# PrivEimantas/myFYP

Measured on AMD Instinct MI355X. Metric: rounds/sec + wall-clock-to-target-acc, MNIST MLP FedAvg 8 peers at 1/2/4/8 MI355X, higher is better.
Workload: dtype fp32

## Files before the change

csrc/kernels/mlp_persistent.h:

```cpp
#pragma once
#include "mlp_fused.h"

struct MLPPersistBufs {
  bf16* h1x;
  bf16* w2x;
  bf16* dh2x;
  unsigned* flags;
  size_t flag_bytes;
  int* err;
  int plain_ok;
  int plain;
};

bool mlp_persistent_supported(const MLPArgs& a);
size_t mlp_persistent_bytes(int P, int Bpad);
size_t mlp_persistent_flag_bytes(int P);
int mlp_persistent_blocks(int P);
hipError_t mlp_persistent_prepare(const MLPArgs& a);
hipError_t mlp_launch_persistent_epoch(const MLPArgs& a, const MLPPersistBufs& pb, hipStream_t s, bool zero_flags = true);

struct MLPPersistF32Bufs {
  float* h1x;
  float* plx;
  float* dh2x;
  unsigned* gen;
  unsigned* flags;
  size_t flag_bytes;
  int* err;
  unsigned fbase;
  float* w2chk;
  int plain_ok;
  int plain;
  int plain_x;
  int c2_straight;
  int k24;
};

int mlp_plain_pub_mode();
bool mlp_persistent_f32_supported(const MLPArgs& a);
size_t mlp_persistent_f32_h1x_floats(int P, int Bpad);
size_t mlp_persistent_f32_bytes(int P, int Bpad);
size_t mlp_persistent_f32_flag_bytes(int P);
int mlp_persistent_f32_gang();
int mlp_persistent_f32_resident_capacity(const MLPArgs& a, int num_cus);
int mlp_persistent_f32_launch_wgs(const MLPArgs& a);
int mlp_persistent_f32_ks(const MLPArgs& a);
int mlp_persistent_f32_variant(const MLPArgs& a);
int mlp_persistent_f32_flags_per_peer();
void mlp_persistent_f32_flag_layout(int* line, int* lines_per_peer, int* full_lines);
hipError_t mlp_persistent_f32_prepare(const MLPArgs& a);
hipError_t mlp_launch_persistent_f32_epoch(const MLPArgs& a, const MLPPersistF32Bufs& pb, hipStream_t s, bool zero_flags = true,
                                           const int* active = nullptr);
void mlp_launch_eval_f32(const MLPArgs& a, int max_rows, hipStream_t s);
```

csrc/kernels/mlp_persistent_f32.hip:

```cpp
#include <atomic>

#include "mlp_persistent.h"
#include "persist_common.h"
#include "mlp_f32_common.h"

bool mlp_f32v2_supported(const MLPArgs& a);
size_t mlp_f32v2_lds(const MLPArgs& a);
size_t mlp_f32v2_bytes(int P, int Bpad);
int mlp_f32v2_launch_wgs();
int mlp_f32v2_resident_capacity(const MLPArgs& a, int num_cus);
hipError_t mlp_f32v2_prepare(const MLPArgs& a);
void mlp_f32v2_launch(const MLPArgs& a, const MLPPersistF32Bufs& pb, hipStream_t s);

#ifdef MLP_STAMPS
__device__ unsigned long long g_p32_stamps[2][128][18];
__device__ unsigned long long g_p32_epoch[4];
#define P32_STAMP(role, t, i)                                                                    \
  do {                                                                                           \
    if (p == 0 && threadIdx.x == 0 && (t) < 128) g_p32_stamps[role][t][i] = wall_clock64(); \
  } while (0)
#define P32_ESTAMP(i)                                        \
  do {                                                       \
    if (p == 0 && threadIdx.x == 0) g_p32_epoch[i] = wall_clock64(); \
  } while (0)
// ... 183 lines not shown
    if (q == RQ && (KS != 1 || s >= KS1)) break;
#pragma unroll
    for (int half = 0; half < 2; ++half) {
      const int k = C0 + 32 * s + 16 * half + 4 * h;
      float4 wv = {0.f, 0.f, 0.f, 0.f}, mv = wv, vv = wv, ev = wv;
      if (s < KS1 && k < D0) {
        const int64_t idx = pS + a.off_w1 + (int64_t)orow * D0 + k;
        wv = *reinterpret_cast<const float4*>(a.params + idx);
        if (!fresh) {
          mv = *reinterpret_cast<const float4*>(a.m + idx);
          if (ADAM) vv = *reinterpret_cast<const float4*>(a.v + idx);
        }
        if (EXTRA) ev = float4{extra_at(a, idx), extra_at(a, idx + 1), extra_at(a, idx + 2), extra_at(a, idx + 3)};
      } else if (s < KS1 && k == D0) {
        const int64_t idx = pS + a.off_b1 + orow;
        wv.x = a.params[idx];
        if (!fresh) {
          mv.x = a.m[idx];
          if (ADAM) vv.x = a.v[idx];
        }
        if (EXTRA) ev.x = extra_at(a, idx);
      }
      if (q < RQ) {
        const float wa[4] = {wv.x, wv.y, wv.z, wv.w}, ma[4] = {mv.x, mv.y, mv.z, mv.w}, va[4] = {vv.x, vv.y, vv.z, vv.w},
                    ea[4] = {ev.x, ev.y, ev.z, ev.w};
#pragma unroll
        for (int i = 0; i < 4; ++i) {
          w1[q][4 * half + i] = wa[i];
          m1[q][4 * half + i] = ma[i];
          v1[q][4 * half + i] = va[i];
          e1[q][4 * half + i] = ea[i];
        }
      } else {
        const int off = c * 32 + 16 * half + 4 * h;
        *reinterpret_cast<float4*>(sW1x + off) = wv;
        *reinterpret_cast<float4*>(sW1x + 512 + off) = mv;
        *reinterpret_cast<float4*>(sW1x + 1024 + off) = vv;
        *reinterpret_cast<float4*>(sW1x + 1536 + off) = ev;
      }
    }
  }
  float w2c[4], m2c[4], v2c[4], e2c[4];
#pragma unroll
  for (int i = 0; i < 4; ++i) {
    const int64_t idx = pS + a.off_w2 + (int64_t)(16 * wave + 4 * h + i) * PD1 + NCG * cg + c;
    w2c[i] = a.params[idx];
    m2c[i] = fresh ? 0.f : a.m[idx];
    v2c[i] = (ADAM && !fresh) ? a.v[idx] : 0.f;
    e2c[i] = EXTRA ? extra_at(a, idx) : 0.f;
  }

  auto bias_chunk = [](bool valid) { return uint4{valid ? 0x3F80u : 0u, 0u, 0u, 0u}; };
  auto xw_stage = [&](int t, int lv) {
    const int rows = rows_at(a, n, t);
#pragma unroll
    for (int k = 0; k < XPT; ++k) {
      const int q = k / (BP / 16), kk = k % (BP / 16);
      if (q > RQ || (q == RQ && KS != 1)) break;
      const int s = wave + 8 * q;
      const int idx = kk * 64 + lv;
      const int r = idx >> 2, col = 32 * s + 8 * (idx & 3), gcol = C0 + col;
      if (s < KS1 && gcol < D0) {
        const bf16* src = a.Xb16 + ((int64_t)p * a.xb_rows + (int64_t)t * a.B + r) * D0 + gcol;
        *reinterpret_cast<uint4*>(sX + r * LDX + col) = r < rows ? *reinterpret_cast<const uint4*>(src) : uint4{0u, 0u, 0u, 0u};
      } else if (s < KS1 && gcol == D0) {
        *reinterpret_cast<uint4*>(sX + r * LDX + col) = bias_chunk(r < rows);
      }
    }
  };
  {
    const int z0 = D0 - C0 + 8, z1 = KS1 * 32;
    if (z0 < z1)
      for (int e = tid; e < BP * (z1 - z0); e += NT) {
        const int r = e / (z1 - z0), q = e % (z1 - z0);
        sX[r * LDX + (z0 + q)] = (bf16)0.f;
      }
  }
  if (nsteps > 0) xw_stage(0, lane);

  auto w2_replica_update = [&](int tp, float lr_p, float inv_p) {
    const __amdgpu_buffer_rsrc_t rd = rsrc_of(pb.dh2x + ((int64_t)p * 2 + (tp & 1)) * BP * PD2 * 2, BP * PD2 * 8);
    int lr = lane;
    asm volatile("" : "+v"(lr));
    const int ro = 4 * ((lr >> 4) * PD2 + 16 * wave + (lr & 15));
    const float* h1p = sH1 + (tp & 1) * BP * 16;
    float av[BP / 4];
#pragma unroll
    for (int kb = 0; kb < BP / 4; ++kb) av[kb] = __builtin_bit_cast(float, __builtin_amdgcn_raw_buffer_load_b32(rd, ro + 4 * 4 * kb * PD2, 0, 16));
    f32x4 acc = zero4();
#pragma unroll
    for (int kb = 0; kb < BP / 4; ++kb) acc = mfma_f32(av[kb], h1p[(4 * kb + h) * 16 + c], acc);
#pragma unroll
    for (int i = 0; i < 4; ++i) upd32<ADAM, EXTRA>(o, acc[i], w2c[i], m2c[i], v2c[i], e2c[i], lr_p, inv_p, wdmu);
  };
  auto fwd_kstep = [&](int q, f32x4(&acc)[MT], bool chk = true, bool rx = false) __attribute__((always_inline)) {
    const int s = wave + 8 * q;
    if (chk && s >= KS1) return;
    int lq = lane;
    asm volatile("" : "+v"(lq));
    const int hq = lq >> 4, cq = lq & 15;
    float wq[8];
#pragma unroll
    for (int j = 0; j < 8; ++j) wq[j] = q < RQ ? w1[q < RQ ? q : 0][j] : rx ? w1x[j] : sW1x[cq * 32 + kappa(hq, j)];
    bf16x8 bh, bm, bl;
    split3(wq, bh, bm, bl);
    if constexpr (FUSE) {
      bf16x8 af[MT];
#pragma unroll
      for (int mt = 0; mt < MT; ++mt) {
        const bf16* xp = sX + (16 * mt + cq) * LDX + 32 * s + 4 * (hq & 1);
        af[mt] = cat8(*reinterpret_cast<const bf16x4*>(xp + ((hq >> 1) << 3)), *reinterpret_cast<const bf16x4*>(xp + ((2 + (hq >> 1)) << 3)));
      }
#pragma unroll
      for (int mt = 0; mt < MT; ++mt) acc[mt] = mfma_bf16(af[mt], bl, acc[mt]);
#pragma unroll
      for (int mt = 0; mt < MT; ++mt) acc[mt] = mfma_bf16(af[mt], bm, acc[mt]);
#pragma unroll
      for (int mt = 0; mt < MT; ++mt) acc[mt] = mfma_bf16(af[mt], bh, acc[mt]);
      return;
    }
#pragma unroll
    for (int mt = 0; mt < MT; ++mt) {
      const bf16* xp = sX + (16 * mt + cq) * LDX + 32 * s + 4 * (hq & 1);
      const bf16x8 af = cat8(*reinterpret_cast<const bf16x4*>(xp + ((hq >> 1) << 3)), *reinterpret_cast<const bf16x4*>(xp + ((2 + (hq >> 1)) << 3)));
      acc[mt] = mfma3(af, bh, bm, bl, acc[mt]);
    }
  };
  auto fwd_all = [&](f32x4(&acc)[MT]) {
#pragma unroll
    for (int mt = 0; mt < MT; ++mt) acc[mt] = zero4();
#pragma unroll
    for (int q = 0; q < (KS == 1 ? RQ + 1 : RQ); ++q) {
      fwd_kstep(q, acc);
      __builtin_amdgcn_sched_barrier(0);
    }
  };
  auto h1_publish = [&](int t, const f32x4(&acc)[MT]) -> bool {
    const int rows = rows_at(a, n, t);
    float* sH1c = sH1 + (t & 1) * BP * 16;
    int tq = tid;
    asm volatile("" : "+v"(tq));
#pragma unroll
    for (int mt = 0; mt < MT; ++mt) sRed[(wave * MT + mt) * 64 + (tq & 63)] = acc[mt];
    lds_barrier();
    if (tq < MT * 64) {
      const int mt = tq >> 6, hh = (tq & 63) >> 4, cc = tq & 15;
      f32x4 s = sRed[mt * 64 + (tq & 63)];
#pragma unroll
      for (int w = 1; w < 8; ++w) s += sRed[(w * MT + mt) * 64 + (tq & 63)];
#pragma unroll
      for (int i = 0; i < 4; ++i) {
        const int b = 16 * mt + 4 * hh + i;
        const float v = b < rows ? (KS == 1 ? fmaxf(s[i], 0.f) : s[i]) : 0.f;
        sH1c[b * 16 + cc] = v;
        persist::pub32(pb.plain, h1x_part(pb, p, kh, t, BP) + (unsigned)(b * PD1 + NCG * cg + cc), v);
      }
    }
    if (g == 0) P32_STAMP(0, t, 1);
    persist::publish_p(pb.flags, FPP, p, XR ? F_H1P + cg * KS + kh : F_H1 + g, pb.fbase + (unsigned)(t + 1), pb.plain);
    if (XR) {
      if (!persist::wg_wait(pb.flags, FPP, p, F_H1P + cg * KS, KS, pb.fbase + (unsigned)(t + 1), pb.err, sOk)) return false;
      if (tid < BP * 4) {
        const int b = tid >> 2, c4 = 4 * (tid & 3);
        float4 u[KS];
#pragma unroll
        for (int k2 = 0; k2 < KS; ++k2)
          u[k2] = k2 == kh ? *reinterpret_cast<const float4*>(sH1c + b * 16 + c4)
                           : ld_sc1_16(rsrc_of(h1x_part(pb, p, k2, t, BP), BP * PD1 * 4), (b * PD1 + NCG * cg + c4) * 4);
        float4 sum = u[0];
#pragma unroll
        for (int k2 = 1; k2 < KS; ++k2) {
// ... 62 lines not shown
    const unsigned t1 = (unsigned)(t + 1);
    bc.next(o, lr_t, inv_bc2);
    float* sH1c = sH1 + (t & 1) * BP * 16;
    if (g == 0) P32_STAMP(0, t, 0);

    if constexpr (!FUSE) {
      f32x4 acc[MT];
      fwd_all(acc);
      if (g == 0) P32_STAMP(0, t, 7);
      if (!h1_publish(t, acc)) return;
    }

    if (!RH && t > 0) w2_replica_update(t - 1, lr_prev, inv_prev);
    if (g == 0) P32_STAMP(0, t, 3);

    const bool more = t + 1 < nsteps;
    if (more) {
      const int rows_n = rows_at(a, n, t + 1);
      unsigned sink = 0;
      int xi = lane;
      if (FUSE) asm volatile("" : "+v"(xi));
      const bf16* xbase = a.Xb16 + ((int64_t)p * a.xb_rows + (int64_t)(t + 1) * a.B) * D0;
      const bf16* xrow = xbase + (unsigned)(xi * D0);
#pragma unroll
      for (int q = 0; q < (KS == 1 ? RQ + 1 : RQ); ++q) {
        const int s = wave + 8 * q;
        const int r = lane;
        if (s < KS1 && C0 + 32 * s < D0 && r < rows_n && r < BP)
          sink ^= *reinterpret_cast<const unsigned*>(xrow + C0 + 32 * s);
      }
      asm volatile("" ::"v"(sink));
    }

    constexpr int XQF = FUSE ? BP / 16 : 1;
    uint4 xqf[XQF];
    const __amdgpu_buffer_rsrc_t r_xn =
        rsrc_of(a.Xb16 + ((int64_t)p * a.xb_rows + (int64_t)(t + 1) * a.B) * D0, more ? rows_at(a, n, t + 1) * D0 * 2 : 0);
    auto xq_load = [&](int q, bool chk = true) __attribute__((always_inline)) {
      const int s = wave + 8 * q;
      if (chk && s >= KS1) return;
      int lx = lane;
      if (chk)
        asm volatile("" : "+v"(lx));
      else
        lx = tv & 63;
#pragma unroll
      for (int kk = 0; kk < XQF; ++kk) {
        const int idx = kk * 64 + lx;
        const int r = idx >> 2, gcol = C0 + 32 * s + 8 * (idx & 3);
        unsigned off = (unsigned)(r * D0 + gcol) * 2u;
        asm("" : "+v"(off));
        off = gcol < D0 ? off : 0x7FFFFFF0u;
        asm("" : "+v"(off));
        xqf[kk] = __builtin_bit_cast(uint4, __builtin_amdgcn_raw_buffer_load_b128(r_xn, off, 0, 0));
      }
    };
    if constexpr (FUSE) xq_load(0);

    const float* dh2_t = pb.dh2x + ((int64_t)p * 2 + (t & 1)) * BP * PD2 * 2;
    const __amdgpu_buffer_rsrc_t r_dh2 = rsrc_of(dh2_t, BP * PD2 * 8);
    if (!persist::wg_wait(pb.flags, FPP, p, RH ? F3_DH2 : F_DH2, RH ? nhr_of(BP) : NH, pb.fbase + t1, pb.err, sOk)) return;
    if (g == 0) P32_STAMP(0, t, 4);
    if (KS > 1 && !XR) {
      if (tid < BP * 4) {
        const int b = tid >> 2, c4 = 4 * (tid & 3);
        float4 sum = {0.f, 0.f, 0.f, 0.f};
#pragma unroll
        for (int k2 = 0; k2 < KS; ++k2) {
          float4 v;
          if (k2 == kh) {
            v = *reinterpret_cast<const float4*>(sH1c + b * 16 + c4);
          } else {
            const __amdgpu_buffer_rsrc_t r = rsrc_of(h1x_part(pb, p, k2, t, BP), BP * PD1 * 4);
            v = ld_sc1_16(r, (b * PD1 + NCG * cg + c4) * 4);
          }
          sum.x += v.x;
          sum.y += v.y;
          sum.z += v.z;
          sum.w += v.w;
        }
        *reinterpret_cast<float4*>(sH1c + b * 16 + c4) = float4{fmaxf(sum.x, 0.f), fmaxf(sum.y, 0.f), fmaxf(sum.z, 0.f), fmaxf(sum.w, 0.f)};
      }
    }
    {
      float4 v[BP / 16];
#pragma unroll
      for (int k = 0; k < BP / 16; ++k) v[k] = ld_sc1_16(r_dh2, (tv + NT * k) * 16);
#pragma unroll
      for (int k = 0; k < BP / 16; ++k) {
        const int e = tv + NT * k;
        *reinterpret_cast<float4*>(sDH2 + (e >> 5) * LDD + 4 * (e & 31)) = v[k];
      }
    }
    lds_barrier();
    if (sOk[1] == 0) return;
    {
      f32x4 acc1[MT];
#pragma unroll
      for (int mt = 0; mt < MT; ++mt) {
        const float4 av = *reinterpret_cast<const float4*>(sDH2 + (16 * mt + c) * LDD + 16 * wave + 4 * h);
        f32x4 acc = mfma_f32(av.x, w2c[0], zero4());
        acc = mfma_f32(av.y, w2c[1], acc);
        acc = mfma_f32(av.z, w2c[2], acc);
        acc1[mt] = mfma_f32(av.w, w2c[3], acc);
      }
      f32x4 dw2 = zero4();
      if (RH) {
        const float* h1p = sH1c;
#pragma unroll
        for (int kb = 0; kb < BP / 4; ++kb) dw2 = mfma_f32(sDH2[(4 * kb + h) * LDD + 16 * wave + c], h1p[(4 * kb + h) * 16 + c], dw2);
      }
      lds_barrier();
#pragma unroll
      for (int mt = 0; mt < MT; ++mt) sRed[(wave * MT + mt) * 64 + lane] = acc1[mt];
      if (RH) {
#pragma unroll
        for (int i = 0; i < 4; ++i) upd32<ADAM, EXTRA>(o, dw2[i], w2c[i], m2c[i], v2c[i], e2c[i], lr_t, inv_bc2, wdmu);
        if (kh == 0) {
          float* w2x = pb.dh2x + (int64_t)a.P * 2 * BP * PD2 * 2 + (int64_t)p * PD2 * PD1;
#pragma unroll
          for (int i = 0; i < 4; ++i) persist::pub32(pb.plain, w2x + (16 * wave + 4 * h + i) * PD1 + NCG * cg + c, w2c[i]);
        }
      }
    }
    if (RH && kh == 0) {
      persist::publish_p(pb.flags, FPP, p, F3_W2 + cg, pb.fbase + (unsigned)(t + 2), pb.plain);
    } else {
      lds_barrier();
    }
    if (tv < MT * 64) {
      const int mt = tv >> 6, hh = (tv & 63) >> 4, cc = tv & 15;
      f32x4 s = sRed[mt * 64 + (tv & 63)];
#pragma unroll
      for (int w = 1; w < 8; ++w) s += sRed[(w * MT + mt) * 64 + (tv & 63)];
      bf16x4 dh, dm, dl;
#pragma unroll
      for (int i = 0; i < 4; ++i) {
        const float d = sH1c[(16 * mt + 4 * hh + i) * 16 + cc] > 0.f ? s[i] : 0.f;
        const bf16 x0 = (bf16)d;
        const float r = d - (float)x0;
        const bf16 x1 = (bf16)r;
        dh[i] = x0;
        dm[i] = x1;
        dl[i] = (bf16)(r - (float)x1);
      }
      const int off = cc * LDT + 16 * mt + 4 * hh;
      *reinterpret_cast<bf16x4*>(sD3 + off) = dh;
      *reinterpret_cast<bf16x4*>(sD3 + 16 * LDT + off) = dm;
      *reinterpret_cast<bf16x4*>(sD3 + 32 * LDT + off) = dl;
    }
    lds_barrier();
    if (g == 0) P32_STAMP(0, t, 5);
    {
      int lv = lane;
      asm volatile("" : "+v"(lv));
      f32x4 accF[FUSE ? MT : 1];
#pragma unroll
      for (int mt = 0; mt < (FUSE ? MT : 1); ++mt) accF[mt] = zero4();
      const int rows_next = more ? rows_at(a, n, t + 1) : 0;
      const bf16* xnext = a.Xb16 + ((int64_t)p * a.xb_rows + (int64_t)(t + 1) * a.B) * D0;
      constexpr int DFR = FUSE ? BP / 32 : 1;
      bf16x8 dfr[3][DFR];
      if (FUSE && ST) {
        int lq = lane;
        asm volatile("" : "+v"(lq));
        const bf16* dfrag = sD3 + (lq & 15) * LDT + 8 * (lq >> 4);
#pragma unroll
        for (int kb = 0; kb < DFR; ++kb) {
          dfr[0][kb] = ld8(dfrag + 32 * kb);
          dfr[1][kb] = ld8(dfrag + 16 * LDT + 32 * kb);
          dfr[2][kb] = ld8(dfrag + 32 * LDT + 32 * kb);
        }
      }
#pragma unroll
      for (int q = 0; q < QN; ++q) {
        if (q >= qn) continue;
        const bool STq = ST && (q < RQ || KR);
        const int s = wave + 8 * q;
        if (STq || s < KS1) {
          int lq = lane;
          asm volatile("" : "+v"(lq));
          const bf16* dfrag = sD3 + (lq & 15) * LDT + 8 * (lq >> 4);
          constexpr int XQ = BP / 16;
          uint4 xq[XQ];
#pragma unroll
          for (int kk = 0; kk < XQ; ++kk) {
            if constexpr (FUSE) {
              xq[kk] = xqf[FUSE ? kk : 0];
              continue;
            }
            const int idx = kk * 64 + lv;
            const int r = idx >> 2, col = 32 * s + 8 * (idx & 3), gcol = C0 + col;
            if (STq) {
              unsigned off = (unsigned)(r * D0 + gcol) * 2u;
              asm("" : "+v"(off));
// ... 301 lines not shown
          acc[mt] = mfma_f32(av.x, w2[gg][0], acc[mt]);
          acc[mt] = mfma_f32(av.y, w2[gg][1], acc[mt]);
          acc[mt] = mfma_f32(av.z, w2[gg][2], acc[mt]);
          acc[mt] = mfma_f32(av.w, w2[gg][3], acc[mt]);
        }
      }
#pragma unroll
      for (int mt = 0; mt < MT; ++mt) sRed[(wave * MT + mt) * 64 + lane] = acc[mt];
    }
    lds_barrier();
    if (tid < MT * 64) {
      const int mt = tid >> 6, hh = (tid & 63) >> 4, cc = tid & 15;
      f32x4 s = sRed[mt * 64 + (tid & 63)];
#pragma unroll
      for (int w = 1; w < 8; ++w) s += sRed[(w * MT + mt) * 64 + (tid & 63)];
      const float bias = sB2[cc];
#pragma unroll
      for (int i = 0; i < 4; ++i) {
        const int b = 16 * mt + 4 * hh + i;
        sH2[b * LD16 + cc] = b < rows ? fmaxf(s[i] + bias, 0.f) : 0.f;
      }
    }
    lds_barrier();
    if (wave < MT) {
      const float4 av = *reinterpret_cast<const float4*>(sH2 + (16 * wave + c) * LD16 + 4 * h);
      const float4 bv = *reinterpret_cast<const float4*>(sW3 + c * LD16 + 4 * h);
      f32x4 pl = mfma_f32(av.x, bv.x, zero4());
      pl = mfma_f32(av.y, bv.y, pl);
      pl = mfma_f32(av.z, bv.z, pl);
      pl = mfma_f32(av.w, bv.w, pl);
      persist::pub128(pb.plain, pb.plx + ((int64_t)p * NH + hd) * BP * 16 * 2, BP * 16 * 4, (wave * 64 + lane) * 16, __builtin_bit_cast(u32x4, pl));
    }
    if (hd == 0) P32_STAMP(1, t, 3);
    persist::publish_p(pb.flags, FPP, p, F_PL + hd, target, pb.plain);
    if (!persist::wg_wait(pb.flags, FPP, p, F_PL, NH, target, pb.err, sOk)) return;
    if (hd == 0) P32_STAMP(1, t, 4);

    if (wave < SMW) {
      float lsum[SMR];
      const __amdgpu_buffer_rsrc_t r = rsrc_of(pb.plx + (int64_t)p * NH * BP * 16 * 2, NH * BP * 16 * 8);
      float uf[NH][SMR];
#pragma unroll
      for (int k = 0; k < NH; ++k) {
        const int off = k * BP * 16 * 8 + (sm_mt * 64 + lane) * 16 + sm_i0 * 4;
        static_assert(SMR == 2, "one 8-byte load per head");
        const u32x2 v = __builtin_amdgcn_raw_buffer_load_b64(r, off, 0, 16);
        uf[k][0] = __uint_as_float(v[0]);
        uf[k][1] = __uint_as_float(v[1]);
      }
      if (hd == 0) P32_STAMP(1, t, 5);
#pragma unroll
      for (int i = 0; i < SMR; ++i) {
        float sv = uf[0][i];
#pragma unroll
        for (int k = 1; k < NH; ++k) sv += uf[k][i];
        lsum[i] = sv;
      }
      const float b3 = sB3[c];
#pragma unroll
      for (int i = 0; i < SMR; ++i) {
        const int b = 16 * sm_mt + 4 * h + sm_i0 + i;
        const bool rvalid = b < rows;
        const int y = yv[i];
        const float logit = cin ? lsum[i] + b3 : -INFINITY;
        const float mx = row_max16(logit);
        const float ex = cin ? __expf(logit - mx) : 0.f;
        const float se = row_sum16(ex);
        const float logp = logit - (mx + __logf(se));
        cand_v[i] = (cin && logit == mx) ? c : 16;
        if (rvalid && c == y) loss_acc -= logp;
        const float pc = ex * __builtin_amdgcn_rcpf(se);
        const float others = row_sum16(c != y ? pc : 0.f);
        sDlog[b * LD16 + c] = (rvalid && cin) ? (c == y ? -others : pc) / (float)rows : 0.f;
      }
    }
    lds_barrier();
    if (sOk[1] == 0) return;
    if (hd == 0) P32_STAMP(1, t, 6);
    if (wave < MT) {
      f32x4 acc = zero4();
#pragma unroll
      for (int ks = 0; ks < 4; ++ks) acc = mfma_f32(sDlog[(16 * wave + c) * LD16 + 4 * ks + h], sW3[(4 * ks + h) * LD16 + c], acc);
      float* dst = pb.dh2x + ((int64_t)p * 2 + (t & 1)) * BP * PD2 * 2;
#pragma unroll
      for (int i = 0; i < 4; ++i) {
        const int b = 16 * wave + 4 * h + i;
        const float v = sH2[b * LD16 + c] > 0.f ? acc[i] : 0.f;
        sDH2[b * LD16 + c] = v;
        persist::pub32(pb.plain_x, dst + b * PD2 + 16 * hd + c, v);
      }
    }
    persist::publish_p(pb.flags, FPP, p, F_DH2 + hd, target, pb.plain_x);
    if (hd == 0) P32_STAMP(1, t, 7);
    if (wave < SMW) {
#pragma unroll
      for (int i = 0; i < SMR; ++i) {
        const int b = 16 * sm_mt + 4 * h + sm_i0 + i;
        const int cand = row_min16(cand_v[i]);
        if (b < rows && c == 0) correct_acc += (cand == yv[i]) ? 1.f : 0.f;
      }
    }

#pragma unroll
    for (int gg = 0; gg < 2; ++gg) {
      const int g = 2 * wave + gg;
      f32x4 acc = zero4();
#pragma unroll
      for (int kb = 0; kb < BP / 4; ++kb) acc = mfma_f32(sH1[(4 * kb + h) * LDH1 + 16 * g + c], sDH2[(4 * kb + h) * LD16 + c], acc);
#pragma unroll
      for (int i = 0; i < 4; ++i) upd32<ADAM, EXTRA>(o, acc[i], w2[gg][i], m2[gg][i], v2[gg][i], e2[gg][i], lr_t, inv_bc2, wdmu);
    }
    if (wave == 0) {
      f32x4 acc = zero4();
#pragma unroll
      for (int kb = 0; kb < BP / 4; ++kb) acc = mfma_f32(sH2[(4 * kb + h) * LD16 + c], sDlog[(4 * kb + h) * LD16 + c], acc);
      if (cin) {
#pragma unroll
        for (int i = 0; i < 4; ++i) {
          upd32<ADAM, EXTRA>(o, acc[i], w3[i], m3[i], v3[i], e3[i], lr_t, inv_bc2, wdmu);
          sW3[c * LD16 + 4 * h + i] = w3[i];
        }
      }
    } else if (wave == 1) {
      f32x4 acc = zero4();
#pragma unroll
      for (int kb = 0; kb < BP / 4; ++kb) acc = mfma_f32(1.f, sDH2[(4 * kb + h) * LD16 + c], acc);
      if (lane < 16) upd32<ADAM, EXTRA>(o, acc[0], sB2[c], sB2[16 + c], sB2[32 + c], sB2[48 + c], lr_t, inv_bc2, wdmu);
    } else if (wave == 2) {
      f32x4 acc = zero4();
#pragma unroll
      for (int kb = 0; kb < BP / 4; ++kb) acc = mfma_f32(1.f, sDlog[(4 * kb + h) * LD16 + c], acc);
      if (lane < 16 && cin) upd32<ADAM, EXTRA>(o, acc[0], sB3[c], sB3[16 + c], sB3[32 + c], sB3[48 + c], lr_t, inv_bc2, wdmu);
    }
    __syncthreads();
    if (hd == 0) P32_STAMP(1, t, 8);
  }

  if (!gang_commit<KS, false, BP>(a, pb, p, ng_of(KS) + hd, sOk)) return;
#pragma unroll
  for (int gg = 0; gg < 2; ++gg) {
    const int64_t idx = pS + a.off_w2 + (int64_t)o2 * PD1 + 16 * (2 * wave + gg) + 4 * h;
    *reinterpret_cast<float4*>(a.params + idx) = float4{w2[gg][0], w2[gg][1], w2[gg][2], w2[gg][3]};
    *reinterpret_cast<float4*>(a.m + idx) = float4{m2[gg][0], m2[gg][1], m2[gg][2], m2[gg][3]};
    if (ADAM) *reinterpret_cast<float4*>(a.v + idx) = float4{v2[gg][0], v2[gg][1], v2[gg][2], v2[gg][3]};
  }
  if (wave == 0 && cin) {
    const int64_t idx = pS + a.off_w3 + (int64_t)c * PD2 + 16 * hd + 4 * h;
#pragma unroll
    for (int i = 0; i < 4; ++i) {
      a.params[idx + i] = w3[i];
      a.m[idx + i] = m3[i];
      if (ADAM) a.v[idx + i] = v3[i];
    }
  }
  if (tid < 16) {
    const int64_t idx = pS + a.off_b2 + 16 * hd + tid;
    a.params[idx] = sB2[tid];
    a.m[idx] = sB2[16 + tid];
    if (ADAM) a.v[idx] = sB2[32 + tid];
  } else if (hd == 0 && tid >= 64 && tid < 64 + D3) {
    const int k = tid - 64;
    const int64_t idx = pS + a.off_b3 + k;
    a.params[idx] = sB3[k];
    a.m[idx] = sB3[16 + k];
    if (ADAM) a.v[idx] = sB3[32 + k];
  }
  if (hd == 0 && wave < MT * (4 / SMR)) {
    const float l = wave_sum(loss_acc), cr = wave_sum(correct_acc);
    if (lane == 0) {
      atomicAdd(&a.loss_acc[p], l);
      atomicAdd(&a.correct_acc[p], (int)(cr + 0.5f));
    }
// ... 709 lines not shown
  hipError_t e;
  for (int KS = 1; KS <= KSMAX; KS *= 2) {
    const int lds = (int)persistent_f32_lds_ks(a, KS);
    if (KS > 2) {
      if (a.Bpad != 64) continue;
      e = KS == 4 ? prepare_f32_bp<64, 4>(lds) : prepare_f32_bp<64, 8>(lds);
      if (e != hipSuccess) return e;
      continue;
    }
    e = KS == 1 ? (a.Bpad == 64 ? prepare_f32_bp<64, 1>(lds) : prepare_f32_bp<32, 1>(lds))
                : (a.Bpad == 64 ? prepare_f32_bp<64, 2>(lds) : prepare_f32_bp<32, 2>(lds));
    if (e != hipSuccess) return e;
    if (v3_supported(a)) {
      const int l3 = (int)persistent_f32_lds_ks(a, KS, true);
      e = KS == 1 ? (a.Bpad == 64 ? prepare_f32_bp<64, 1, true>(l3) : prepare_f32_bp<32, 1, true>(l3))
                  : (a.Bpad == 64 ? prepare_f32_bp<64, 2, true>(l3) : prepare_f32_bp<32, 2, true>(l3));
      if (e != hipSuccess) return e;
    }
  }
  if (mlp_f32v2_supported(a)) {
    e = mlp_f32v2_prepare(a);
    if (e != hipSuccess) return e;
  }
  return hipFuncSetAttribute((const void*)mlp_eval_f32, hipFuncAttributeMaxDynamicSharedMemorySize, (int)eval_lds32(a.D0));
}

static std::atomic<int> g_plain_override{-1};
int mlp_plain_pub_mode() {
  const int o = g_plain_override.load(std::memory_order_relaxed);
  if (o >= 0) return o;
  static const int v = [] {
    const char* e = getenv("MYFYP_F32_PLAIN_PUB");
    return e != nullptr ? atoi(e) : 1;
  }();
  return v;
}
extern "C" int mlp_set_plain_pub(int mode) { return g_plain_override.exchange(mode < 0 ? -1 : mode); }
extern "C" int mlp_debug_plain_seen(int* out) {
  return hipMemcpyFromSymbol(out, HIP_SYMBOL(g_plain_seen), sizeof(g_plain_seen)) == hipSuccess ? 0 : 1;
}

static std::atomic<int> g_fuse_override{-1};
static std::atomic<int> g_fuse_last{-1};
static int f32_fwd_fuse_mode() {
  const int o = g_fuse_override.load(std::memory_order_relaxed);
  if (o >= 0) return o;
  static const int v = [] {
    const char* e = getenv("MYFYP_F32_FWD_FUSE");
    return e != nullptr ? atoi(e) : 1;
  }();
  return v;
}
extern "C" int mlp_set_f32_fwd_fuse(int mode) { return g_fuse_override.exchange(mode < 0 ? -1 : mode); }
extern "C" int mlp_f32_fwd_fuse_last() { return g_fuse_last.load(std::memory_order_relaxed); }

static std::atomic<int> g_straight_override{-1};
static std::atomic<int> g_straight_last{-1};
static int f32_c2_straight_mode() {
  const int o = g_straight_override.load(std::memory_order_relaxed);
  if (o >= 0) return o;
  static const int v = [] {
    const char* e = getenv("MYFYP_F32_C2_STRAIGHT");
    return e != nullptr ? atoi(e) : 1;
  }();
  return v;
}
extern "C" int mlp_set_f32_c2_straight(int mode) { return g_straight_override.exchange(mode < 0 ? -1 : mode); }
extern "C" int mlp_f32_c2_straight_last() { return g_straight_last.load(std::memory_order_relaxed); }

static std::atomic<int> g_k24_override{-1};
static std::atomic<int> g_k24_last{-1};
static int f32_k24_mode() {
  const int o = g_k24_override.load(std::memory_order_relaxed);
  if (o >= 0) return o;
  static const int v = [] {
    const char* e = getenv("MYFYP_F32_K24");
    return e != nullptr ? atoi(e) : 1;
  }();
  return v;
}
extern "C" int mlp_set_f32_k24(int mode) { return g_k24_override.exchange(mode < 0 ? -1 : mode); }
extern "C" int mlp_f32_k24_last() { return g_k24_last.load(std::memory_order_relaxed); }

hipError_t mlp_launch_persistent_f32_epoch(const MLPArgs& a, const MLPPersistF32Bufs& pb_in, hipStream_t s, bool zero_flags, const int* active) {
  MLPPersistF32Bufs pb = pb_in;
  pb.plain_ok = mlp_plain_pub_mode();
  pb.plain = 0;
  if (zero_flags) {
    hipError_t e = hipMemsetAsync(pb.flags, 0, pb.flag_bytes, s);
    if (e != hipSuccess) return e;
  }
  if (f32_variant(a) == 2) {
    mlp_f32v2_launch(a, pb, s);
    return hipGetLastError();
  }
  const int KS = f32_ks(a);
  const bool rh = f32_variant(a) == 3;
  const int ppl = ppl_of(KS, rh);
  const size_t lds = persistent_f32_lds_ks(a, KS, rh);
  const bool fuse = f32_fwd_fuse_mode() != 0 && fuse_inst(KS, rh) && a.anchor == nullptr && a.cg == nullptr;
  g_fuse_last.store(fuse ? 1 : 0, std::memory_order_relaxed);
  pb.c2_straight = f32_c2_straight_mode() != 0 ? 1 : 0;
  const bool straight_all = pb.c2_straight && !rh && KS == 1 && 7 + 8 * (rq_of(1) - 1) < ks1_of(a.D0);
  g_straight_last.store(straight_all ? 1 : 0, std::memory_order_relaxed);
  pb.k24 = f32_k24_mode() > 0 && fuse && straight_all && 8 * rq_of(1) < ks1_of(a.D0) ? 1 : 0;
  g_k24_last.store(pb.k24, std::memory_order_relaxed);
  auto group_live = [&](int p0) {
    if (active == nullptr) return true;
    for (int p = p0; p < p0 + ppl && p < a.P; ++p)
      if (active[p]) return true;
    return false;
  };
  for (int attempt = 0; attempt < 2; ++attempt)
    for (int p0 = 0; p0 < a.P; p0 += ppl) {
      if (!group_live(p0)) continue;
      if (rh) {
        if (KS == 2) {
          if (a.Bpad == 64) launch_f32_bp<64, 2, true>(a, pb, s, p0, lds, attempt, fuse);
          else launch_f32_bp<32, 2, true>(a, pb, s, p0, lds, attempt, fuse);
        } else {
          if (a.Bpad == 64) launch_f32_bp<64, 1, true>(a, pb, s, p0, lds, attempt, fuse);
          else launch_f32_bp<32, 1, true>(a, pb, s, p0, lds, attempt, fuse);
        }
      } else if (KS == 8) {
        launch_f32_bp<64, 8>(a, pb, s, p0, lds, attempt, fuse);
      } else if (KS == 4) {
        launch_f32_bp<64, 4>(a, pb, s, p0, lds, attempt, fuse);
      } else if (KS == 2) {
        if (a.Bpad == 64) launch_f32_bp<64, 2>(a, pb, s, p0, lds, attempt, fuse);
        else launch_f32_bp<32, 2>(a, pb, s, p0, lds, attempt, fuse);
      } else {
        if (a.Bpad == 64) launch_f32_bp<64, 1>(a, pb, s, p0, lds, attempt, fuse);
        else launch_f32_bp<32, 1>(a, pb, s, p0, lds, attempt, fuse);
      }
    }
  return hipGetLastError();
}

static int eval_wgs_cap() {
  static const int v = [] {
    const char* e = getenv("MYFYP_EVAL_WGS");
    return e != nullptr ? atoi(e) : 32;
  }();
  return v;
}
void mlp_launch_eval_f32(const MLPArgs& a, int max_rows, hipStream_t s) {
  if (max_rows <= 0) return;
  const int chunks = (max_rows + EV_ROWS - 1) / EV_ROWS, cap = eval_wgs_cap();
  const int per_peer = cap > 0 ? (cap / a.P > 0 ? cap / a.P : 1) : chunks;
  const dim3 grid(chunks < per_peer ? chunks : per_peer, a.P);
  hipLaunchKernelGGL(mlp_eval_f32, grid, dim3(NT), eval_lds32(a.D0), s, a);
}

extern "C" int myfyp_warm_mlp_f32() {
  hipFuncAttributes attr;
  return hipFuncGetAttributes(&attr, reinterpret_cast<const void*>(&mlp_eval_f32)) == hipSuccess ? 0 : 1;
}
```

myfyp_amd/ops/_native.py:

```python

from __future__ import annotations

import ctypes
import os
import threading
from typing import Optional

_LIB: Optional[ctypes.CDLL] = None
_FAST: Optional[ctypes.PyDLL] = None
_LOCK = threading.Lock()
_ERR: Optional[str] = None

LIB_DIR = os.path.join(os.path.dirname(os.path.dirname(os.path.abspath(__file__))), "_native")
LIB_PATH = os.environ.get("MYFYP_NATIVE_LIB") or os.path.join(LIB_DIR, "libmyfyp_hip.so")

c_void_p = ctypes.c_void_p
c_int = ctypes.c_int
c_int64 = ctypes.c_int64
c_float = ctypes.c_float

_SIGNATURES = {
    "myfyp_version": (c_int, []),
    "myfyp_last_error": (ctypes.c_char_p, []),
    "myfyp_weighted_sum": (c_int, [c_void_p, c_void_p, c_void_p, c_int, c_int64, c_int, c_void_p]),
    "myfyp_stacked_weighted_sum": (c_int, [c_void_p, c_void_p, c_int, c_int64, c_int64, c_void_p, c_float, c_void_p]),
    "myfyp_broadcast_rows": (c_int, [c_void_p, c_void_p, c_int, c_int64, c_int64, c_void_p, c_void_p]),
    "myfyp_coordinate_median": (c_int, [c_void_p, c_void_p, c_int, c_int64, c_void_p]),
    "myfyp_coordinate_median_multi": (c_int, [c_void_p, c_int, c_void_p, c_int, c_int64, c_void_p]),
    "myfyp_trimmed_mean_multi": (c_int, [c_void_p, c_int, c_void_p, c_int, c_int, c_int64, c_void_p]),
    "myfyp_krum_grid": (c_int, [c_int64, c_int]),
    "myfyp_krum_multi": (c_int, [c_void_p, c_int, c_void_p, c_void_p, c_int, c_int, c_int, c_int64, c_void_p, c_void_p, c_void_p, c_void_p, c_void_p]),
    "myfyp_bulyan_multi": (c_int, [c_void_p, c_int, c_void_p, c_int, c_int, c_int64, c_void_p, c_void_p, c_void_p, c_void_p, c_void_p, c_void_p]),
    "myfyp_bulyan_mean_multi": (c_int, [c_void_p, c_int, c_void_p, c_int, c_int, c_int64, c_void_p, c_void_p]),
    "myfyp_geomed_work": (c_int64, [c_int64, c_int]),
    "myfyp_geomed_multi": (c_int, [c_void_p, c_int, c_void_p, c_void_p, c_int, c_int, ctypes.c_double, c_int64, c_void_p, c_void_p, c_void_p, c_void_p, c_void_p]),
    "myfyp_scaffold_reduce": (c_int, [c_void_p, c_void_p, c_void_p, c_void_p, c_int, c_int64, c_void_p]),
    "myfyp_scaffold_apply": (c_int, [c_void_p, c_int, c_void_p, c_void_p, c_void_p, c_int, c_float, c_int64, c_void_p]),
    "myfyp_adam_step": (
        c_int,
        [c_void_p, c_void_p, c_void_p, c_void_p, c_void_p, c_int64, c_float, c_float, c_float, c_float, c_float, c_int, c_void_p, c_void_p, c_void_p, c_float, c_void_p],
    ),
    "myfyp_sgd_step": (c_int, [c_void_p, c_void_p, c_void_p, c_int64, c_float, c_float, c_float, c_int, c_void_p, c_void_p, c_void_p, c_float, c_void_p]),
    "myfyp_scale_add_noise": (c_int, [c_void_p, c_int64, c_float, c_float, ctypes.c_uint64, c_void_p]),

    "mlp_shape_ok": (c_int, [c_int, c_int, c_int, c_int]),
    "mlp_engine_create": (c_void_p, [c_int, c_int, c_int, c_int, c_int, c_int]),
    "mlp_engine_destroy": (None, [c_void_p]),
    "mlp_engine_numel": (c_int64, [c_void_p]),
    "mlp_engine_bind_params": (c_int, [c_void_p, c_void_p, c_void_p, c_void_p, c_void_p, c_void_p, c_int64]),
    "mlp_engine_set_train_data": (c_int, [c_void_p, c_void_p, c_void_p, c_void_p, c_void_p, c_int64, c_int]),
    "mlp_engine_set_test_data": (c_int, [c_void_p, c_void_p, c_void_p, c_void_p, c_int]),
    "mlp_engine_set_counts": (c_int, [c_void_p, c_void_p, c_void_p]),
    "mlp_engine_set_optimizer": (c_int, [c_void_p, c_int, c_float, c_float, c_float, c_float, c_float, c_float, c_int, c_float]),
    "mlp_engine_set_extras": (c_int, [c_void_p, c_void_p, c_void_p, c_void_p]),
    "mlp_engine_begin": (c_int, [c_void_p, c_void_p, c_void_p]),
    "mlp_engine_run_epoch": (c_int, [c_void_p, c_void_p, c_void_p]),
    "mlp_engine_run_epoch_pub": (c_int, [c_void_p, c_void_p, c_int, c_void_p]),
    "mlp_engine_drain_prep": (c_int, [c_void_p]),
    "mlp_engine_run_epoch_eager": (c_int, [c_void_p, c_void_p, c_void_p]),
    "mlp_engine_read_stats": (c_int, [c_void_p, c_void_p, c_void_p, c_void_p]),
    "mlp_engine_eval": (c_int, [c_void_p, c_void_p, c_void_p, c_void_p, c_void_p, c_void_p]),
    "mlp_engine_stats_async": (c_int, [c_void_p, c_int, c_void_p]),
    "mlp_engine_eval_async": (c_int, [c_void_p, c_void_p, c_int, c_void_p]),
    "mlp_engine_fetch": (c_int, [c_void_p, c_int, c_void_p, c_void_p, c_void_p]),
    "mlp_engine_ring_size": (c_int, []),
    "mlp_engine_set_persistent": (c_int, [c_void_p, c_int]),
    "mlp_engine_zero_state": (c_int, [c_void_p, c_void_p]),
    "mlp_engine_set_shuffle": (c_int, [c_void_p, c_int]),
    "mlp_engine_set_epoch_seed": (c_int, [c_void_p, ctypes.c_uint64]),
    "mlp_engine_set_next_epoch_seed": (c_int, [c_void_p, ctypes.c_uint64]),
    "myfyp_fedavg_stacked_reduce": (c_int, [c_void_p, c_void_p, c_int, c_int64, c_int64, c_void_p, c_void_p]),
    "myfyp_fedavg_stacked_apply": (c_int, [c_void_p, c_void_p, c_int, c_int64, c_int64, c_void_p, c_void_p]),
    "myfyp_fedavg_stacked_local": (c_int, [c_void_p, c_int, c_int64, c_int64, c_void_p, c_void_p, c_void_p]),
    "myfyp_fedavg_bucket_reduce": (c_int, [c_void_p, c_void_p, c_void_p, c_int, c_int64, c_int64, c_void_p, c_void_p]),
    "myfyp_fedavg_bucket_apply": (c_int, [c_void_p, c_void_p, c_void_p, c_int, c_int64, c_int64, c_void_p, c_void_p]),
    "myfyp_fedavg_bucket_reduce2": (c_int, [c_void_p, c_void_p, c_void_p, c_void_p, c_void_p, c_int, c_int64, c_int64, c_void_p, c_void_p]),
    "myfyp_fedavg_delayed_land": (c_int, [c_void_p, c_void_p, c_int64, c_void_p, c_void_p, c_int, c_int64, c_int64, c_void_p, c_void_p]),
    "myfyp_neighbor_mix_stacked": (c_int, [c_void_p, c_int, c_int64, c_int64, c_void_p, c_void_p]),
    "mlp_engine_uses_persistent": (c_int, [c_void_p]),
    "mlp_engine_set_precision": (c_int, [c_void_p, c_int]),
    "mlp_f32_ok": (c_int, [c_int, c_int, c_int, c_int, c_int]),
    "mlp_engine_set_w2chk": (c_int, [c_void_p, c_void_p]),
    "mlp_engine_recoveries": (c_int, [c_void_p]),
    "mlp_engine_graph_launch_stats": (c_int, [c_void_p, c_void_p]),
    "mlp_engine_set_f32_ks": (c_int, [c_void_p, c_int]),
    "mlp_engine_set_reserved_cus": (c_int, [c_void_p, c_int]),
    "mlp_engine_f32_ks": (c_int, [c_void_p]),
    "mlp_engine_set_f32_variant": (c_int, [c_void_p, c_int]),
    "mlp_engine_f32_variant": (c_int, [c_void_p]),
    "mlp_engine_debug_giveup": (c_int, [c_void_p, c_int, c_int]),
    "mlp_engine_debug_poison_flags": (c_int, [c_void_p, c_int]),
    "mlp_engine_prepare": (c_int, [c_void_p, c_void_p]),
    "myfyp_warm_all": (c_int, [c_int]),
    "mlp_set_plain_pub": (c_int, [c_int]),
    "mlp_debug_plain_seen": (c_int, [c_void_p]),
    "mlp_set_f32_fwd_fuse": (c_int, [c_int]),
    "mlp_f32_fwd_fuse_last": (c_int, []),
    "mlp_set_f32_c2_straight": (c_int, [c_int]),
    "mlp_f32_c2_straight_last": (c_int, []),
    "mlp_set_f32_k24": (c_int, [c_int]),
    "mlp_f32_k24_last": (c_int, []),
    "mlp_debug_stamps": (c_int, [c_void_p]),
    "mlp_debug_persistent_f32_stamps": (c_int, [c_void_p]),
}


def load(required: bool = False) -> Optional[ctypes.CDLL]:
    global _LIB, _ERR
    if _LIB is not None:
        return _LIB
    with _LOCK:
        if _LIB is None and _ERR is None:
            if not os.path.exists(LIB_PATH):
                _ERR = f"native library not built: {LIB_PATH} (run python -m myfyp_amd.ops.build)"
            else:
                try:
                    lib = ctypes.CDLL(LIB_PATH, mode=ctypes.RTLD_GLOBAL)
                    for name, (res, args) in _SIGNATURES.items():
                        fn = getattr(lib, name, None)
                        if fn is None:
                            continue
                        fn.restype = res
                        fn.argtypes = args
                    _LIB = lib
                except OSError as e:
                    _ERR = f"failed to load {LIB_PATH}: {e}"
    if _LIB is None and required:
        raise RuntimeError(_ERR or "native library unavailable")
    return _LIB


def load_fast() -> ctypes.PyDLL:
    global _FAST
    if _FAST is not None:
        return _FAST
    load(required=True)
    with _LOCK:
        if _FAST is None:
            lib = ctypes.PyDLL(LIB_PATH, mode=ctypes.RTLD_GLOBAL)
            for name, (res, args) in _SIGNATURES.items():
                fn = getattr(lib, name, None)
                if fn is None:
                    continue
                fn.restype = res
                fn.argtypes = args
            _FAST = lib
    return _FAST


def debug_update_scale() -> float:
    v = os.environ.get("MYFYP_DEBUG_LR_SCALE")
    return float(v) if v else 1.0


_WARM: set = set()


def warm_device(index: int, family: str = "mlp") -> None:
    key = (index, family)
    if key in _WARM:
        return
    lib = load(required=True)
    fn = getattr(lib, "myfyp_warm_all", None)
    if fn is not None:
        bad = int(fn(1 if family == "mlp" else 2))
        if bad:
            raise RuntimeError(f"native code objects: {bad} kernel unit(s) failed to load on device {index}")
    _WARM.add(key)


def available() -> bool:
    return load() is not None


def error() -> Optional[str]:
    load()
    return _ERR


def check(rc: int, what: str) -> None:
    if rc != 0:
        msg = _LIB.myfyp_last_error().decode() if _LIB is not None else "?"
        raise RuntimeError(f"{what} failed (rc={rc}): {msg}")
```

Measured before the change: 739.5.

## Publish dh2 exchange buffer in MFMA fragment layout to skip LDS staging

Adds a 'frag' layout for the cross-workgroup dh2 exchange buffer: the producer writes dh2 in the exact per-lane MFMA operand order using 128-bit publishes, and consumers load their operand fragments directly from global memory into registers. This removes the LDS staging copy and two workgroup barriers in the backward dh1 step, and changes the W2 replica update's load addressing to match. It is on by default for variant 1 only, behind an env var or setter. The risks are non-coalesced fragment addressing and the extra LDS round trip plus waitcnt the producer needs before its vector publish.

```diff
diff --git a/csrc/kernels/mlp_persistent.h b/csrc/kernels/mlp_persistent.h
--- a/csrc/kernels/mlp_persistent.h
+++ b/csrc/kernels/mlp_persistent.h
@@ -34,6 +34,7 @@
   int plain_x;
   int c2_straight;
   int k24;
+  int dh2_frag;
 };
 
 int mlp_plain_pub_mode();
diff --git a/csrc/kernels/mlp_persistent_f32.hip b/csrc/kernels/mlp_persistent_f32.hip
--- a/csrc/kernels/mlp_persistent_f32.hip
+++ b/csrc/kernels/mlp_persistent_f32.hip
@@ -289,11 +289,17 @@
     const __amdgpu_buffer_rsrc_t rd = rsrc_of(pb.dh2x + ((int64_t)p * 2 + (tp & 1)) * BP * PD2 * 2, BP * PD2 * 8);
     int lr = lane;
     asm volatile("" : "+v"(lr));
-    const int ro = 4 * ((lr >> 4) * PD2 + 16 * wave + (lr & 15));
     const float* h1p = sH1 + (tp & 1) * BP * 16;
     float av[BP / 4];
-#pragma unroll
-    for (int kb = 0; kb < BP / 4; ++kb) av[kb] = __builtin_bit_cast(float, __builtin_amdgcn_raw_buffer_load_b32(rd, ro + 4 * 4 * kb * PD2, 0, 16));
+    if (!RH && pb.dh2_frag != 0) {
+      const int ro = 4 * (((wave * MT) * 64 + ((lr & 15) >> 2) * 16 + (lr >> 4)) * 4 + (lr & 3));
+#pragma unroll
+      for (int kb = 0; kb < BP / 4; ++kb) av[kb] = __builtin_bit_cast(float, __builtin_amdgcn_raw_buffer_load_b32(rd, ro + 1024 * (kb >> 2) + 64 * (kb & 3), 0, 16));
+    } else {
+      const int ro = 4 * ((lr >> 4) * PD2 + 16 * wave + (lr & 15));
+#pragma unroll
+      for (int kb = 0; kb < BP / 4; ++kb) av[kb] = __builtin_bit_cast(float, __builtin_amdgcn_raw_buffer_load_b32(rd, ro + 4 * 4 * kb * PD2, 0, 16));
+    }
     f32x4 acc = zero4();
 #pragma unroll
     for (int kb = 0; kb < BP / 4; ++kb) acc = mfma_f32(av[kb], h1p[(4 * kb + h) * 16 + c], acc);
@@ -522,7 +528,12 @@
         *reinterpret_cast<float4*>(sH1c + b * 16 + c4) = float4{fmaxf(sum.x, 0.f), fmaxf(sum.y, 0.f), fmaxf(sum.z, 0.f), fmaxf(sum.w, 0.f)};
       }
     }
-    {
+    const bool frag = !RH && pb.dh2_frag != 0;
+    float4 avf[MT];
+    if (frag) {
+#pragma unroll
+      for (int mt = 0; mt < MT; ++mt) avf[mt] = ld_sc1_16(r_dh2, ((wave * MT + mt) * 64 + (tv & 63)) * 16);
+    } else {
       float4 v[BP / 16];
 #pragma unroll
       for (int k = 0; k < BP / 16; ++k) v[k] = ld_sc1_16(r_dh2, (tv + NT * k) * 16);
@@ -531,18 +542,23 @@
         const int e = tv + NT * k;
         *reinterpret_cast<float4*>(sDH2 + (e >> 5) * LDD + 4 * (e & 31)) = v[k];
       }
-    }
-    lds_barrier();
+      lds_barrier();
+    }
     if (sOk[1] == 0) return;
     {
       f32x4 acc1[MT];
-#pragma unroll
-      for (int mt = 0; mt < MT; ++mt) {
-        const float4 av = *reinterpret_cast<const float4*>(sDH2 + (16 * mt + c) * LDD + 16 * wave + 4 * h);
+      auto dh1_chain = [&](const float4 av) __attribute__((always_inline)) {
         f32x4 acc = mfma_f32(av.x, w2c[0], zero4());
         acc = mfma_f32(av.y, w2c[1], acc);
         acc = mfma_f32(av.z, w2c[2], acc);
-        acc1[mt] = mfma_f32(av.w, w2c[3], acc);
+        return mfma_f32(av.w, w2c[3], acc);
+      };
+      if (frag) {
+#pragma unroll
+        for (int mt = 0; mt < MT; ++mt) acc1[mt] = dh1_chain(avf[mt]);
+      } else {
+#pragma unroll
+        for (int mt = 0; mt < MT; ++mt) acc1[mt] = dh1_chain(*reinterpret_cast<const float4*>(sDH2 + (16 * mt + c) * LDD + 16 * wave + 4 * h));
       }
       f32x4 dw2 = zero4();
       if (RH) {
@@ -550,7 +566,7 @@
 #pragma unroll
         for (int kb = 0; kb < BP / 4; ++kb) dw2 = mfma_f32(sDH2[(4 * kb + h) * LDD + 16 * wave + c], h1p[(4 * kb + h) * 16 + c], dw2);
       }
-      lds_barrier();
+      if (!frag) lds_barrier();
 #pragma unroll
       for (int mt = 0; mt < MT; ++mt) sRed[(wave * MT + mt) * 64 + lane] = acc1[mt];
       if (RH) {
@@ -1018,12 +1034,23 @@
 #pragma unroll
       for (int ks = 0; ks < 4; ++ks) acc = mfma_f32(sDlog[(16 * wave + c) * LD16 + 4 * ks + h], sW3[(4 * ks + h) * LD16 + c], acc);
       float* dst = pb.dh2x + ((int64_t)p * 2 + (t & 1)) * BP * PD2 * 2;
-#pragma unroll
-      for (int i = 0; i < 4; ++i) {
-        const int b = 16 * wave + 4 * h + i;
-        const float v = sH2[b * LD16 + c] > 0.f ? acc[i] : 0.f;
-        sDH2[b * LD16 + c] = v;
-        persist::pub32(pb.plain_x, dst + b * PD2 + 16 * hd + c, v);
+      if (pb.dh2_frag != 0) {
+#pragma unroll
+        for (int i = 0; i < 4; ++i) {
+          const int b = 16 * wave + 4 * h + i;
+          sDH2[b * LD16 + c] = sH2[b * LD16 + c] > 0.f ? acc[i] : 0.f;
+        }
+        asm volatile("s_waitcnt lgkmcnt(0)" ::: "memory");
+        const float4 fr = *reinterpret_cast<const float4*>(sDH2 + (16 * wave + c) * LD16 + 4 * h);
+        persist::pub128(pb.plain_x, dst, BP * PD2 * 4, ((hd * MT + wave) * 64 + (tv & 63)) * 16, __builtin_bit_cast(u32x4, fr));
+      } else {
+#pragma unroll
+        for (int i = 0; i < 4; ++i) {
+          const int b = 16 * wave + 4 * h + i;
+          const float v = sH2[b * LD16 + c] > 0.f ? acc[i] : 0.f;
+          sDH2[b * LD16 + c] = v;
+          persist::pub32(pb.plain_x, dst + b * PD2 + 16 * hd + c, v);
+        }
       }
     }
     persist::publish_p(pb.flags, FPP, p, F_DH2 + hd, target, pb.plain_x);
@@ -1899,10 +1926,26 @@
 extern "C" int mlp_set_f32_k24(int mode) { return g_k24_override.exchange(mode < 0 ? -1 : mode); }
 extern "C" int mlp_f32_k24_last() { return g_k24_last.load(std::memory_order_relaxed); }
 
+static std::atomic<int> g_dh2_frag_override{-1};
+static std::atomic<int> g_dh2_frag_last{-1};
+static int f32_dh2_frag_mode() {
+  const int o = g_dh2_frag_override.load(std::memory_order_relaxed);
+  if (o >= 0) return o;
+  static const int v = [] {
+    const char* e = getenv("MYFYP_F32_DH2_FRAG");
+    return e != nullptr ? atoi(e) : 1;
+  }();
+  return v;
+}
+extern "C" int mlp_set_f32_dh2_frag(int mode) { return g_dh2_frag_override.exchange(mode < 0 ? -1 : mode); }
+extern "C" int mlp_f32_dh2_frag_last() { return g_dh2_frag_last.load(std::memory_order_relaxed); }
+
 hipError_t mlp_launch_persistent_f32_epoch(const MLPArgs& a, const MLPPersistF32Bufs& pb_in, hipStream_t s, bool zero_flags, const int* active) {
   MLPPersistF32Bufs pb = pb_in;
   pb.plain_ok = mlp_plain_pub_mode();
   pb.plain = 0;
+  pb.dh2_frag = f32_dh2_frag_mode() > 0 && f32_variant(a) == 1 ? 1 : 0;
+  g_dh2_frag_last.store(pb.dh2_frag, std::memory_order_relaxed);
   if (zero_flags) {
     hipError_t e = hipMemsetAsync(pb.flags, 0, pb.flag_bytes, s);
     if (e != hipSuccess) return e;
diff --git a/myfyp_amd/ops/_native.py b/myfyp_amd/ops/_native.py
--- a/myfyp_amd/ops/_native.py
+++ b/myfyp_amd/ops/_native.py
@@ -100,6 +100,8 @@
     "mlp_f32_c2_straight_last": (c_int, []),
     "mlp_set_f32_k24": (c_int, [c_int]),
     "mlp_f32_k24_last": (c_int, []),
+    "mlp_set_f32_dh2_frag": (c_int, [c_int]),
+    "mlp_f32_dh2_frag_last": (c_int, []),
     "mlp_debug_stamps": (c_int, [c_void_p]),
     "mlp_debug_persistent_f32_stamps": (c_int, [c_void_p]),
 }
```

After: 754.7, median of 6. 1.02x the previous value.
